# kerrm/vlite-fast

Measured on AMD Instinct MI355X. Metric: Msamp/s/antenna (dual-pol) and x real-time @128 MS/s; % HBM roofline, higher is better.
Workload: dtype f32

## Files before the change

### vlite-fast_amd/csrc/search_dev.h

```cpp
#pragma once
#include <hip/hip_runtime.h>

#include <cstdint>

#define GATHER_FLUSH 240

typedef uint32_t gather_u32x4 __attribute__((ext_vector_type(4), aligned(4)));

template <int NDW>
__device__ __forceinline__ void gather_load(const uint32_t *p, uint32_t (&w)[NDW + 1])
{
#pragma unroll
    for (int i = 0; i + 4 <= NDW + 1; i += 4) {
        const gather_u32x4 v = *(const gather_u32x4 *)(p + i);
        w[i] = v.x;
        w[i + 1] = v.y;
        w[i + 2] = v.z;
        w[i + 3] = v.w;
    }
#pragma unroll
    for (int i = (NDW + 1) & ~3; i <= NDW; ++i) w[i] = p[i];
}

template <int NDW>
__device__ __forceinline__ void gather_load_guarded(const uint8_t *xt, long long off, uint32_t (&w)[NDW + 1])
{
    if (off >= 0) {
        gather_load<NDW>((const uint32_t *)(xt + off), w);
    } else {
#pragma unroll
        for (int i = 0; i <= NDW; ++i)
            if (off + 4 * i >= 0) w[i] = *(const uint32_t *)(xt + off + 4 * i);
    }
}

__device__ __forceinline__ uint32_t gather_align(uint32_t w0, uint32_t w1, unsigned sh) { return __builtin_amdgcn_alignbyte(w1, w0, sh); }

template <int NDW>
__device__ __forceinline__ void gather_shift(const uint32_t (&w)[NDW + 1], unsigned sh, uint32_t (&a)[NDW])
{
#pragma unroll
    for (int i = 0; i < NDW; ++i) a[i] = gather_align(w[i], w[i + 1], sh);
}

#define SA_T 64
#define SA_B 64
#define SA_PITCH 84
#define SA_BPITCH 68

__device__ __forceinline__ void stream_store16(uint8_t *__restrict__ row, int td, int lo, int hi, const uint32_t (&w)[4])
{
    if (td >= lo && td + 16 <= hi) {
        *(uint4 *)(row + td) = make_uint4(w[0], w[1], w[2], w[3]);
        return;
    }
#pragma unroll
    for (int q = 0; q < 4; ++q) {
        const int tq = td + 4 * q;
        if (tq >= lo && tq + 4 <= hi) {
            *(uint32_t *)(row + tq) = w[q];
        } else {
#pragma unroll
            for (int k = 0; k < 4; ++k)
                if (tq + k >= lo && tq + k < hi) row[tq + k] = (uint8_t)(w[q] >> (8 * k));
        }
    }
}


template <typename T, typename Op>
__device__ __forceinline__ T block_reduce(T v, T *sh, T zero, Op op)
{
    for (int o = 32; o >= 1; o >>= 1) v = op(v, __shfl_down(v, o));
    __syncthreads();
    if ((threadIdx.x & 63) == 0) sh[threadIdx.x >> 6] = v;
    __syncthreads();
    T r = zero;
#pragma unroll
    for (int i = 0; i < 4; ++i) r = op(r, sh[i]);
    return r;
}

template <typename T>
__device__ __forceinline__ T block_sum(T v, T *sh)
{
    return block_reduce(v, sh, (T)0, [](T a, T b) { return a + b; });
}

__device__ __forceinline__ unsigned long long block_max(unsigned long long v, unsigned long long *sh)
{
    return block_reduce(v, sh, 0ull, [](unsigned long long a, unsigned long long b) { return b > a ? b : a; });
}

template <typename T>
__device__ __forceinline__ T wave_inclusive_sum(T v)
{
    const int lane = threadIdx.x & 63;
    for (int o = 1; o < 64; o <<= 1) {
        const T y = __shfl_up(v, o);
        if (lane >= o) v += y;
    }
    return v;
}

__device__ __forceinline__ int block_wave_offsets(int wave_total, int *sh, int &before)
{
    const int wave = threadIdx.x >> 6;
    __syncthreads();
    if ((threadIdx.x & 63) == 63) sh[wave] = wave_total;
    __syncthreads();
    int tot = 0;
    before = 0;
#pragma unroll
    for (int w = 0; w < 4; ++w) {
        if (w < wave) before += sh[w];
        tot += sh[w];
    }
    return tot;
}

__device__ __forceinline__ int block_count(bool flag, int *sh, int &rank)
{
    const uint64_t m = __ballot(flag);
    int before;
    const int tot = block_wave_offsets(__popcll(m), sh, before);
    rank = before + __popcll(m & ((1ull << (threadIdx.x & 63)) - 1ull));
    return tot;
}
```

### vlite-fast_amd/csrc/search_run.hip

```cpp
#include "search_internal.h"
#include "search_dev.h"

std::string g_search_err;

__global__ __launch_bounds__(256) void k_transpose_codes(const uint8_t *__restrict__ codes, uint8_t *__restrict__ xt,
                                                         int T, int nchan, int nbit, size_t tpitch)
{
    __shared__ uint8_t tile[64][65];
    const int t0 = blockIdx.x * 64, c0 = blockIdx.y * 64;
    const int per = 8 / nbit, maskv = (1 << nbit) - 1;
    for (int i = threadIdx.x; i < 64 * 64; i += 256) {
        const int tt = i / 64, cc = i % 64;
        const int t = t0 + tt, c = c0 + cc;
        uint8_t v = 0;
        if (t < T && c < nchan) {
            const size_t n = (size_t)t * nchan + c;
            v = (codes[n / per] >> (nbit * (n % per))) & maskv;
        }
        tile[tt][cc] = v;
    }
    __syncthreads();
    for (int i = threadIdx.x; i < 64 * 64; i += 256) {
        const int cc = i / 64, tt = i % 64;
        const int t = t0 + tt, c = c0 + cc;
        if (t < T && c < nchan) xt[(size_t)c * tpitch + t] = tile[tt][cc];
    }
}

#ifndef DDM_DB
#define DDM_DB 4
#endif
#ifndef DDM_SAMPLES
#define DDM_SAMPLES 8
#endif
#ifndef DDM_CU
#define DDM_CU 4
#endif
#define DDM_TILE (256 * DDM_SAMPLES)

__global__ __launch_bounds__(256) void k_dedisperse(const uint8_t *__restrict__ xt, const int32_t *__restrict__ chans,
                                                    const int32_t *__restrict__ delay, uint32_t *__restrict__ D,
                                                    int nact, int ndm, int tout, size_t tpitch, size_t dpitch)
{
    const int dm0 = blockIdx.y * DDM_DB;
    const int t = blockIdx.x * DDM_TILE + threadIdx.x * DDM_SAMPLES;
    if (t >= tout) return;
    uint32_t lo[DDM_DB][DDM_SAMPLES / 4], hi[DDM_DB][DDM_SAMPLES / 4];
    uint32_t acc[DDM_DB][DDM_SAMPLES];
    const int32_t *dl[DDM_DB];
#pragma unroll
    for (int j = 0; j < DDM_DB; ++j) {
        dl[j] = delay + (size_t)(dm0 + j < ndm ? dm0 + j : ndm - 1) * nact;
#pragma unroll
        for (int w = 0; w < DDM_SAMPLES / 4; ++w) lo[j][w] = hi[j][w] = 0u;
#pragma unroll
        for (int i = 0; i < DDM_SAMPLES; ++i) acc[j][i] = 0u;
    }
    auto flush = [&]() {
#pragma unroll
        for (int j = 0; j < DDM_DB; ++j) {
#pragma unroll
            for (int w = 0; w < DDM_SAMPLES / 4; ++w) {
                acc[j][4 * w + 0] += lo[j][w] & 0xffffu;
                acc[j][4 * w + 1] += hi[j][w] & 0xffffu;
                acc[j][4 * w + 2] += lo[j][w] >> 16;
                acc[j][4 * w + 3] += hi[j][w] >> 16;
                lo[j][w] = hi[j][w] = 0u;
            }
        }
    };
    auto fetch = [&](int c, int j, uint32_t (&w)[DDM_SAMPLES / 4 + 1], unsigned &sh) {
        const int32_t d = dl[j][c];
        const uint32_t *p = (const uint32_t *)(xt + (size_t)chans[c] * tpitch + t + (d & ~3));
#pragma unroll
        for (int i = 0; i <= DDM_SAMPLES / 4; ++i) w[i] = p[i];
        sh = (unsigned)(d & 3);
    };
    auto add = [&](int j, const uint32_t (&w)[DDM_SAMPLES / 4 + 1], unsigned sh) {
#pragma unroll
        for (int i = 0; i < DDM_SAMPLES / 4; ++i) {
            const uint32_t a = gather_align(w[i], w[i + 1], sh);
            lo[j][i] += a & 0x00ff00ffu;
            hi[j][i] += (a >> 8) & 0x00ff00ffu;
        }
    };
    int c = 0, since = 0;
    for (; c + DDM_CU <= nact; c += DDM_CU) {
        uint32_t w[DDM_CU][DDM_DB][DDM_SAMPLES / 4 + 1];
        unsigned sh[DDM_CU][DDM_DB];
#pragma unroll
        for (int u = 0; u < DDM_CU; ++u)
#pragma unroll
            for (int j = 0; j < DDM_DB; ++j) fetch(c + u, j, w[u][j], sh[u][j]);
#pragma unroll
        for (int u = 0; u < DDM_CU; ++u)
#pragma unroll
            for (int j = 0; j < DDM_DB; ++j) add(j, w[u][j], sh[u][j]);
        since += DDM_CU;
        if (since >= GATHER_FLUSH) {
            flush();
            since = 0;
        }
    }
    for (; c < nact; ++c) {
#pragma unroll
        for (int j = 0; j < DDM_DB; ++j) {
            uint32_t w[DDM_SAMPLES / 4 + 1];
            unsigned sh;
            fetch(c, j, w, sh);
            add(j, w, sh);
        }
    }
    flush();
#pragma unroll
    for (int j = 0; j < DDM_DB; ++j) {
        if (dm0 + j >= ndm) break;
        uint32_t *out = D + (size_t)(dm0 + j) * dpitch + t;
#pragma unroll
        for (int i = 0; i < DDM_SAMPLES; i += 4) {
            if (t + i + 4 <= tout) {
                *(uint4 *)(out + i) = make_uint4(acc[j][i], acc[j][i + 1], acc[j][i + 2], acc[j][i + 3]);
            } else {
                for (int q = 0; q < 4; ++q)
                    if (t + i + q < tout) out[i + q] = acc[j][i + q];
            }
        }
    }
}

__global__ __launch_bounds__(256) void k_prefix(const uint32_t *__restrict__ D, uint64_t *__restrict__ P, int tout,
                                                size_t dpitch, size_t ppitch)
{
    __shared__ uint64_t sh[256];
    const uint32_t *x = D + (size_t)blockIdx.x * dpitch;
    uint64_t *p = P + (size_t)blockIdx.x * ppitch;
    const int per = (tout + 255) / 256;
    const int lo = threadIdx.x * per, hi = min(lo + per, tout);
    uint64_t s = 0;
    for (int t = lo; t < hi; ++t) s += x[t];
    sh[threadIdx.x] = s;
    __syncthreads();
    if (threadIdx.x == 0) {
        uint64_t run = 0;
        for (int i = 0; i < 256; ++i) {
            const uint64_t v = sh[i];
            sh[i] = run;
            run += v;
        }
        p[0] = 0;
    }
    __syncthreads();
    uint64_t run = sh[threadIdx.x];
    for (int t = lo; t < hi; ++t) {
        run += x[t];
        p[t + 1] = run;
    }
}

__device__ __forceinline__ float baseline_at(const uint64_t *__restrict__ p, int t, int W, int tout, float gmean)
{
    if (W <= 0) return gmean;
    int lo = t - W / 2, hi = lo + W;
    if (lo < 0) { lo = 0; hi = min(W, tout); }
    if (hi > tout) { hi = tout; lo = max(0, tout - W); }
    return (float)((double)(p[hi] - p[lo]) / (double)(hi - lo));
}

__global__ __launch_bounds__(256) void k_series_stats(const uint32_t *__restrict__ D, const uint64_t *__restrict__ P,
                                                      float *__restrict__ stats, int tout, int W, size_t dpitch,
                                                      size_t ppitch)
{
    __shared__ double sh[4];
    const uint32_t *x = D + (size_t)blockIdx.x * dpitch;
    const uint64_t *p = P + (size_t)blockIdx.x * ppitch;
    const float gmean0 = (float)((double)p[tout] / (double)tout);
    double s1 = 0, s2 = 0;
    for (int t = threadIdx.x; t < tout; t += 256) {
        const double v = (double)x[t] - (double)baseline_at(p, t, W, tout, gmean0);
        s1 += v;
        s2 += v * v;
    }
    s1 = block_sum(s1, sh);
    s2 = block_sum(s2, sh);
    double mean = s1 / tout, var = s2 / tout - mean * mean;
    double rms = sqrt(var > 0 ? var : 0);
    const double mean1 = mean, rms1 = rms;
    double c1 = 0, cn = 0;
    for (int t = threadIdx.x; t < tout; t += 256) {
        const double v = (double)x[t] - (double)baseline_at(p, t, W, tout, gmean0);
        if (fabs(v - mean1) <= 3 * rms1) {
            c1 += v;
            cn += 1;
        }
    }
    c1 = block_sum(c1, sh);
    cn = block_sum(cn, sh);
    if (cn > 0) {
        mean = c1 / cn;
        double d2 = 0;
        for (int t = threadIdx.x; t < tout; t += 256) {
            const double v = (double)x[t] - (double)baseline_at(p, t, W, tout, gmean0);
            if (fabs(v - mean1) <= 3 * rms1) d2 += (v - mean) * (v - mean);
        }
        d2 = block_sum(d2, sh);
        rms = sqrt(d2 / cn / 0.97330);
    }
    if (threadIdx.x == 0) {
        stats[2 * blockIdx.x] = (float)(W > 0 ? mean : mean + (double)gmean0);
        stats[2 * blockIdx.x + 1] = (float)rms;
    }
}

__global__ __launch_bounds__(256) void k_boxcar(const uint64_t *__restrict__ P, const float *__restrict__ stats,
                                                float *__restrict__ snr, uint8_t *__restrict__ wid, int tout,
                                                int nbox, int W, size_t dpitch, size_t ppitch, float thresh,
                                                int32_t *__restrict__ peaks, int max_peaks)
{
    const int dm = blockIdx.y;
    const int t = blockIdx.x * 256 + threadIdx.x;
    if (t >= tout) return;
    const uint64_t *p = P + (size_t)dm * ppitch;
    const float lvl = stats[2 * dm], rms = stats[2 * dm + 1];
    float best = -1e30f;
    int bw = 0;
    for (int k = 0; k < nbox; ++k) {
        const int w = 1 << k;
        if (t + w > tout) break;
        const float sum = (float)(p[t + w] - p[t]);
        const float base = W > 0 ? baseline_at(p, t + w / 2, W, tout, 0.f) + lvl : lvl;
        const float sn = (sum - (float)w * base) / (rms * sqrtf((float)w));
        if (sn > best) {
            best = sn;
            bw = k;
        }
    }
    if (!(rms > 0)) best = 0.f;
    snr[(size_t)dm * dpitch + t] = best;
    wid[(size_t)dm * dpitch + t] = (uint8_t)bw;
    if (peaks && best >= thresh) {
        const int i = atomicAdd(peaks, 1);
        if (i < max_peaks) {
            peaks[1 + 4 * i] = dm;
            peaks[2 + 4 * i] = t;
            peaks[3 + 4 * i] = __float_as_int(best);
            peaks[4 + 4 * i] = bw;
        }
    }
}


__device__ __forceinline__ int first_bin_reaching(const uint32_t (&a)[4], uint32_t need)
{
    const int lane = threadIdx.x & 63;
    const uint32_t loc = a[0] + a[1] + a[2] + a[3];
    const uint32_t inc = wave_inclusive_sum(loc);
    const int first = __builtin_ctzll(__ballot(inc >= need));
    uint32_t c = inc - loc;
    int k = 3;
    for (int j = 0; j < 4; ++j) {
        c += a[j];
        if (c >= need) {
            k = j;
            break;
        }
    }
    return __shfl(4 * lane + k, first);
}

__global__ __launch_bounds__(256) void k_rfi_narrow(uint8_t *__restrict__ xt, const int32_t *__restrict__ chans,
                                                    uint8_t *__restrict__ med_out, int nsamp, size_t tpitch, float tol,
                                                    int replace, unsigned long long *__restrict__ nflag)
{
    __shared__ uint32_t hist[4][256];
    __shared__ uint32_t tot[256];
    __shared__ int sh_med, sh_mad;
    __shared__ uint32_t sh_cnt[4];
    const int wave = threadIdx.x >> 6, lane = threadIdx.x & 63;
    for (int i = threadIdx.x; i < 4 * 256; i += 256) hist[i >> 8][i & 255] = 0u;
    __syncthreads();
    uint8_t *row = xt + (size_t)chans[blockIdx.x] * tpitch;
    uint4 *rv = (uint4 *)row;
    const int nvec = nsamp >> 4;
    for (int i = threadIdx.x; i < nvec; i += 256) {
        const uint4 v = rv[i];
        const uint32_t w[4] = {v.x, v.y, v.z, v.w};
#pragma unroll
        for (int j = 0; j < 4; ++j)
#pragma unroll
            for (int b = 0; b < 4; ++b) atomicAdd(&hist[wave][(w[j] >> (8 * b)) & 255u], 1u);
    }
    for (int t = 16 * nvec + threadIdx.x; t < nsamp; t += 256) atomicAdd(&hist[wave][row[t]], 1u);
    __syncthreads();
    tot[threadIdx.x] = hist[0][threadIdx.x] + hist[1][threadIdx.x] + hist[2][threadIdx.x] + hist[3][threadIdx.x];
    __syncthreads();
    if (wave == 0) {
        const uint32_t need = (uint32_t)(nsamp + 1) / 2;
        uint32_t a[4];
#pragma unroll
        for (int j = 0; j < 4; ++j) a[j] = tot[4 * lane + j];
        const int med = first_bin_reaching(a, need);
#pragma unroll
        for (int j = 0; j < 4; ++j) {
            const int d = 4 * lane + j;
            a[j] = d == 0 ? tot[med] : (med - d >= 0 ? tot[med - d] : 0u) + (med + d < 256 ? tot[med + d] : 0u);
        }
        const int mad = first_bin_reaching(a, need);
        if (lane == 0) {
            sh_med = med;
            sh_mad = mad;
            med_out[blockIdx.x] = (uint8_t)med;
        }
    }
    __syncthreads();
    if (!replace) return;
    const int med = sh_med;
    const float thr = tol * 1.4826f * (float)max(sh_mad, 1);
    const int dlim = thr >= 255.f ? 255 : (int)floorf(thr);
    const uint32_t mb = (uint32_t)med;
    uint32_t cnt = 0;
    for (int i = threadIdx.x; i < nvec; i += 256) {
        const uint4 v = rv[i];
        uint32_t w[4] = {v.x, v.y, v.z, v.w};
        uint32_t changed = 0;
#pragma unroll
        for (int j = 0; j < 4; ++j) {
            uint32_t o = 0;
#pragma unroll
            for (int b = 0; b < 4; ++b) {
                const uint32_t x = (w[j] >> (8 * b)) & 255u;
                const bool f = abs((int)x - med) > dlim;
                cnt += f;
                changed |= f;
                o |= (f ? mb : x) << (8 * b);
            }
            w[j] = o;
        }
        if (changed) rv[i] = make_uint4(w[0], w[1], w[2], w[3]);
    }
    for (int t = 16 * nvec + threadIdx.x; t < nsamp; t += 256) {
        if (abs((int)row[t] - med) > dlim) {
            row[t] = (uint8_t)med;
            ++cnt;
        }
    }
    cnt = block_sum(cnt, sh_cnt);
    if (threadIdx.x == 0 && cnt) atomicAdd(nflag, (unsigned long long)cnt);
}

__global__ __launch_bounds__(256) void k_rfi_broad_list(const float *__restrict__ snr, const uint8_t *__restrict__ wid,
                                                        int nsamp, float tol, int widest, int32_t *__restrict__ tlist,
                                                        unsigned long long *__restrict__ nbroad)
{
    __shared__ int end[256 + 64];
    const int base = blockIdx.x * 256;
    for (int i = threadIdx.x; i < 256 + 64; i += 256) {
        const int t0 = base - 64 + i;
        int e = 0;
        if (t0 >= 0 && t0 < nsamp && snr[t0] >= tol) e = t0 + (1 << wid[t0]);
        end[i] = e;
    }
    __syncthreads();
    const int t = base + threadIdx.x;
    if (t >= nsamp) return;
    bool f = false;
    for (int k = 0; k < widest; ++k) f |= end[64 + threadIdx.x - k] > t;
    if (f) {
        const unsigned long long i = atomicAdd(nbroad, 1ull);
        tlist[i] = t;
    }
}

__global__ __launch_bounds__(256) void k_rfi_broad_mask(uint8_t *__restrict__ xt, const int32_t *__restrict__ chans,
                                                        const uint8_t *__restrict__ med, const int32_t *__restrict__ tlist,
                                                        const unsigned long long *__restrict__ nbroad, int nact,
                                                        size_t tpitch)
{
    const int k = blockIdx.x * 4 + (threadIdx.x >> 6);
    if (k >= nact) return;
    const int n = (int)*nbroad;
    uint8_t *row = xt + (size_t)chans[k] * tpitch;
    const uint8_t m = med[k];
    for (int i = threadIdx.x & 63; i < n; i += 64) row[tlist[i]] = m;
}

extern "C" const char *pb_search_last_error(const pb_search *s) { return s ? s->err.c_str() : g_search_err.c_str(); }

static int search_create(int device, int nchan, int max_samples, float fch1_mhz, float foff_mhz, float tsamp_s,
                         const std::vector<double> &dms, int boxcar_max, const int *zap_ranges, int nzap,
                         pb_search **out);

extern "C" int pb_search_create(int device, int nchan, int max_samples, float fch1_mhz, float foff_mhz, float tsamp_s,
                                float dm_min, float dm_max, float dm_step, int boxcar_max, const int *zap_ranges,
                                int nzap, pb_search **out)
{
    if (!out || !(dm_step > 0) || dm_max < dm_min) return search_fail(nullptr, "pb_search_create", "bad argument");
    const int ndm = (int)floor((dm_max - dm_min) / dm_step + 1e-6) + 1;
    std::vector<double> dms(ndm);
    for (int i = 0; i < ndm; ++i) dms[i] = (double)dm_min + (double)i * (double)dm_step;
    return search_create(device, nchan, max_samples, fch1_mhz, foff_mhz, tsamp_s, dms, boxcar_max, zap_ranges, nzap, out);
}

extern "C" int pb_search_create_list(int device, int nchan, int max_samples, float fch1_mhz, float foff_mhz,
                                     float tsamp_s, const float *dm_list, int ndm, int boxcar_max,
                                     const int *zap_ranges, int nzap, pb_search **out)
{
    if (!out || !dm_list || ndm < 1) return search_fail(nullptr, "pb_search_create_list", "bad argument");
    std::vector<double> dms(dm_list, dm_list + ndm);
    for (int i = 1; i < ndm; ++i)
        if (!(dms[i] > dms[i - 1])) return search_fail(nullptr, "pb_search_create_list", "the DM list must be strictly ascending");
    return search_create(device, nchan, max_samples, fch1_mhz, foff_mhz, tsamp_s, dms, boxcar_max, zap_ranges, nzap, out);
}

static int search_create(int device, int nchan, int max_samples, float fch1_mhz, float foff_mhz, float tsamp_s,
                         const std::vector<double> &dms, int boxcar_max, const int *zap_ranges, int nzap,
                         pb_search **out)
{
    const float dm_min = (float)dms.front();
    if (!out || nchan < 1 || max_samples < 64 || boxcar_max < 1) return search_fail(nullptr, "pb_search_create", "bad argument");
    if (!(dm_min >= 0) || device < 0) {
        g_search_err = "pb_search_create: dm_min and device must be >= 0";
        return PB_EINVAL;
    }
    *out = nullptr;
    int ndev = 0;
    if (hipGetDeviceCount(&ndev) != hipSuccess || ndev <= 0 || device >= ndev) {
        g_search_err = "pb_search_create: no HIP device (no CPU fallback)";
        return PB_EHIP;
    }
    pb_search *s = new pb_search();
    s->device = device;
    s->nchan = nchan;
    s->max_samples = max_samples;
    s->fch1 = fch1_mhz;
    s->foff = foff_mhz;
    s->tsamp = tsamp_s;
    s->ndm = (int)dms.size();
    while ((1 << s->nbox) <= boxcar_max) s->nbox++;
    s->dm_last = dms.back();
    std::vector<int32_t> chans;
    for (int c = 0; c < nchan; ++c) {
        bool zap = false;
        for (int z = 0; z < nzap; ++z)
            if (c >= zap_ranges[2 * z] && c < zap_ranges[2 * z + 1]) zap = true;
        if (!zap) chans.push_back(c);
    }
    s->nact = (int)chans.size();
    if (s->nact == 0) {
        g_search_err = "pb_search_create: every channel is zapped";
        delete s;
        return PB_EINVAL;
    }
    std::vector<int32_t> delay((size_t)s->ndm * s->nact);
    const double ftop = foff_mhz < 0 ? fch1_mhz : fch1_mhz + (nchan - 1) * foff_mhz;
    s->ftop = ftop;
    int maxd = 0;
    for (int i = 0; i < s->ndm; ++i) {
        const double dm = dms[i];
        for (int k = 0; k < s->nact; ++k) {
            const double f = (double)fch1_mhz + (double)chans[k] * (double)foff_mhz;
            const int32_t di = delay_samples(dm, delay_chan_term(f, ftop), (double)tsamp_s);
            delay[(size_t)i * s->nact + k] = di;
            if (di > maxd) maxd = di;
        }
    }
    s->max_delay = maxd;
    s->tpitch = ((size_t)max_samples + 63) / 64 * 64;
    hipError_t e = hipSetDevice(device);
    if (e == hipSuccess) e = hipStreamCreateWithFlags(&s->stream, hipStreamNonBlocking);
    if (e == hipSuccess) e = hipMalloc((void **)&s->d_codes, (size_t)max_samples * nchan);
    if (e == hipSuccess) e = hipMalloc((void **)&s->d_xt, s->tpitch * nchan + 64);
    if (e == hipSuccess) e = hipMemset(s->d_xt, 0, s->tpitch * nchan + 64);
    if (e == hipSuccess) e = hipMalloc((void **)&s->d_delay, delay.size() * sizeof(int32_t));
    if (e == hipSuccess) e = hipMalloc((void **)&s->d_chans, chans.size() * sizeof(int32_t));
    if (e == hipSuccess) e = hipMemcpy(s->d_chans, chans.data(), chans.size() * sizeof(int32_t), hipMemcpyHostToDevice);
    if (e == hipSuccess) e = hipMalloc((void **)&s->d_D, (size_t)s->ndm * s->tpitch * sizeof(uint32_t));
    if (e == hipSuccess) e = hipMalloc((void **)&s->d_stats, (size_t)s->ndm * 2 * sizeof(float));
    if (e == hipSuccess) e = hipMalloc((void **)&s->d_snr, (size_t)s->ndm * s->tpitch * sizeof(float));
    if (e == hipSuccess) e = hipMalloc((void **)&s->d_wid, (size_t)s->ndm * s->tpitch);
    if (e == hipSuccess) e = hipMalloc((void **)&s->d_P, (size_t)s->ndm * s->ppitch() * sizeof(uint64_t));
    if (e == hipSuccess) e = hipMalloc((void **)&s->d_peaks, (size_t)(1 + 4 * s->max_peaks) * sizeof(int32_t));
    for (int i = 0; i < 7 && e == hipSuccess; ++i) e = hipEventCreate(&s->ev[i]);
    if (e == hipSuccess) e = hipMemcpy(s->d_delay, delay.data(), delay.size() * sizeof(int32_t), hipMemcpyHostToDevice);
    if (e != hipSuccess) {
        g_search_err = std::string("pb_search_create: ") + hipGetErrorString(e);
        pb_search_destroy(s);
        return PB_EHIP;
    }
    *out = s;
    return PB_OK;
}

void search_rfi_free(pb_search *s)
{
    search_release({s->rfi.d_zdelay, s->rfi.d_med, s->rfi.d_z, s->rfi.d_zP, s->rfi.d_zstats, s->rfi.d_zsnr, s->rfi.d_zwid,
                    s->rfi.d_tlist, s->rfi.d_rcnt}, nullptr, s->rfi.ev, 1);
    s->rfi = {};
}

extern "C" void pb_search_destroy(pb_search *s)
{
    if (!s) return;
    (void)hipSetDevice(s->device);
    if (s->stream) (void)hipStreamSynchronize(s->stream);
    search_rfi_free(s);
    search_rfichan_free(s);
    search_cutouts_free(s);
    search_refine_free(s);
    search_giants_free(s);
    search_gulp_free(s);
    search_pol_free(s);
    search_subbands_free(s);
    search_release({s->d_codes, s->d_xt, s->d_delay, s->d_D, s->d_stats, s->d_snr, s->d_wid, s->d_P, s->d_peaks, s->d_chans},
                   nullptr, s->ev, 7);
    if (s->stream) (void)hipStreamDestroy(s->stream);
    delete s;
}

extern "C" int pb_search_info(const pb_search *s, int *ndm, int *nbox, int *max_delay)
{
    if (!s) return PB_EINVAL;
    if (ndm) *ndm = s->ndm;
    if (nbox) *nbox = s->nbox;
    if (max_delay) *max_delay = s->max_delay;
    return PB_OK;
}

extern "C" int pb_search_set_baseline(pb_search *s, int window_samples)
{
    if (!s || window_samples < 0) return PB_EINVAL;
    s->baseline = window_samples;
    return PB_OK;
}

extern "C" int pb_search_set_rfi(pb_search *s, int narrow, int broad, float tol, int rfi_boxcar_max)
{
    const char *fn = "pb_search_set_rfi";
    if (!(tol > 0) || !std::isfinite(tol)) return search_fail(s, fn, "tol must be > 0 and finite");
    if (rfi_boxcar_max < 1 || rfi_boxcar_max > 64 || (rfi_boxcar_max & (rfi_boxcar_max - 1)))
        return search_fail(s, fn, "rfi_boxcar_max must be a power of two in 1..64");
    if (!s) return search_fail(s, fn, "no search handle");
    if ((narrow || broad) && !s->rfi.d_rcnt) {
        const size_t tp = s->tpitch;
        SCHK(s, hipSetDevice(s->device));
        SCHK(s, hipMalloc((void **)&s->rfi.d_zdelay, (size_t)s->nact * sizeof(int32_t)));
        SCHK(s, hipMemset(s->rfi.d_zdelay, 0, (size_t)s->nact * sizeof(int32_t)));
        SCHK(s, hipMalloc((void **)&s->rfi.d_med, (size_t)s->nact));
        SCHK(s, hipMalloc((void **)&s->rfi.d_z, tp * sizeof(uint32_t)));
        SCHK(s, hipMalloc((void **)&s->rfi.d_zP, s->ppitch() * sizeof(uint64_t)));
        SCHK(s, hipMalloc((void **)&s->rfi.d_zstats, 2 * sizeof(float)));
        SCHK(s, hipMalloc((void **)&s->rfi.d_zsnr, tp * sizeof(float)));
        SCHK(s, hipMalloc((void **)&s->rfi.d_zwid, tp));
        SCHK(s, hipMalloc((void **)&s->rfi.d_tlist, tp * sizeof(int32_t)));
        SCHK(s, hipEventCreate(&s->rfi.ev[0]));
        SCHK(s, hipMalloc((void **)&s->rfi.d_rcnt, 2 * sizeof(unsigned long long)));
    }
    s->rfi.narrow = narrow != 0;
    s->rfi.broad = broad != 0;
    s->rfi.tol = tol;
    s->rfi.nbox = 0;
    while ((1 << s->rfi.nbox) <= rfi_boxcar_max) s->rfi.nbox++;
    return PB_OK;
}

static int search_clean(pb_search *s, int nsamp)
{
    const size_t ppitch = s->ppitch();
    SCHK(s, hipMemsetAsync(s->rfi.d_rcnt, 0, 2 * sizeof(unsigned long long), s->stream));
    k_rfi_narrow<<<s->nact, 256, 0, s->stream>>>(s->d_xt, s->d_chans, s->rfi.d_med, nsamp, s->tpitch, s->rfi.tol,
                                                 s->rfi.narrow, s->rfi.d_rcnt);
    if (s->rfi.broad) {
        dim3 gz((nsamp + DDM_TILE - 1) / DDM_TILE, 1);
        k_dedisperse<<<gz, 256, 0, s->stream>>>(s->d_xt, s->d_chans, s->rfi.d_zdelay, s->rfi.d_z, s->nact, 1, nsamp, s->tpitch,
                                                s->tpitch);
        k_prefix<<<1, 256, 0, s->stream>>>(s->rfi.d_z, s->rfi.d_zP, nsamp, s->tpitch, ppitch);
        k_series_stats<<<1, 256, 0, s->stream>>>(s->rfi.d_z, s->rfi.d_zP, s->rfi.d_zstats, nsamp, s->baseline, s->tpitch, ppitch);
        dim3 gb((nsamp + 255) / 256, 1);
        k_boxcar<<<gb, 256, 0, s->stream>>>(s->rfi.d_zP, s->rfi.d_zstats, s->rfi.d_zsnr, s->rfi.d_zwid, nsamp, s->rfi.nbox, s->baseline,
                                            s->tpitch, ppitch, 0.f, nullptr, 0);
        k_rfi_broad_list<<<gb, 256, 0, s->stream>>>(s->rfi.d_zsnr, s->rfi.d_zwid, nsamp, s->rfi.tol, 1 << (s->rfi.nbox - 1),
                                                    s->rfi.d_tlist, s->rfi.d_rcnt + 1);
        k_rfi_broad_mask<<<(s->nact + 3) / 4, 256, 0, s->stream>>>(s->d_xt, s->d_chans, s->rfi.d_med, s->rfi.d_tlist,
                                                                   s->rfi.d_rcnt + 1, s->nact, s->tpitch);
    }
    SCHK(s, hipEventRecord(s->rfi.ev[0], s->stream));
    return PB_OK;
}

void search_series_launch(pb_search *s, const uint32_t *D, uint64_t *P, float *stats, int nrow, int tout)
{
    k_prefix<<<nrow, 256, 0, s->stream>>>(D, P, tout, s->tpitch, s->ppitch());
    k_series_stats<<<nrow, 256, 0, s->stream>>>(D, P, stats, tout, s->baseline, s->tpitch, s->ppitch());
}

void search_boxcar_launch(pb_search *s, const uint64_t *P, const float *stats, float *snr, uint8_t *wid, int nrow, int tout)
{
    k_boxcar<<<dim3((tout + 255) / 256, nrow), 256, 0, s->stream>>>(P, stats, snr, wid, tout, s->nbox, s->baseline, s->tpitch,
                                                                    s->ppitch(), 0.f, nullptr, 0);
}

int search_block(pb_search *s, int nsamp, float thresh, bool want_peaks, bool cleaned)
{
    const int tout = nsamp - s->max_delay;
    s->rfi.ran = s->rfi.narrow || s->rfi.broad;
    s->chan.launched = s->chan.tol > 0 && !cleaned;
    s->chan.ran = s->chan.launched || (s->chan.tol > 0 && s->chan.have);
    if (s->chan.launched) {
        const int rc = search_rfichan_launch(s, nsamp);
        if (rc) return rc;
    }
    if (s->chan.tol > 0 && !s->rfi.ran) SCHK(s, hipEventRecord(s->chan.ev[2], s->stream));
    if (s->rfi.ran && cleaned) {
        SCHK(s, hipEventRecord(s->rfi.ev[0], s->stream));
    } else if (s->rfi.ran) {
        const int rc = search_clean(s, nsamp);
        if (rc) return rc;
    }
    dim3 gd((tout + 255) / 256, s->ndm);
    dim3 gdd((tout + DDM_TILE - 1) / DDM_TILE, (s->ndm + DDM_DB - 1) / DDM_DB);
    k_dedisperse<<<gdd, 256, 0, s->stream>>>(s->d_xt, s->d_chans, s->d_delay, s->d_D, s->nact, s->ndm, tout, s->tpitch, s->tpitch);
    SCHK(s, hipEventRecord(s->ev[3], s->stream));
    const size_t ppitch = s->ppitch();
    k_prefix<<<s->ndm, 256, 0, s->stream>>>(s->d_D, s->d_P, tout, s->tpitch, ppitch);
    k_series_stats<<<s->ndm, 256, 0, s->stream>>>(s->d_D, s->d_P, s->d_stats, tout, s->baseline, s->tpitch, ppitch);
    SCHK(s, hipEventRecord(s->ev[4], s->stream));
    if (want_peaks) SCHK(s, hipMemsetAsync(s->d_peaks, 0, sizeof(int32_t), s->stream));
    k_boxcar<<<gd, 256, 0, s->stream>>>(s->d_P, s->d_stats, s->d_snr, s->d_wid, tout, s->nbox, s->baseline, s->tpitch,
                                        ppitch, thresh, want_peaks ? s->d_peaks : nullptr, s->max_peaks);
    SCHK(s, hipEventRecord(s->ev[5], s->stream));
    SCHK(s, hipGetLastError());
    s->last_tout = tout;
    s->last_nsamp = nsamp;
    s->plane_tout = tout;
    return PB_OK;
}

static int search_run(pb_search *s, const void *codes, int codes_on_device, int nsamp, int nbit, float thresh,
                      bool want_peaks)
{
    if (!s || !codes) return PB_EINVAL;
    if (nsamp > s->max_samples || !(nbit == 8 || nbit == 4 || nbit == 2))
        return search_fail(s, "pb_search_run", "block too long or bad nbit");
    const int tout = nsamp - s->max_delay;
    if (tout < 64) return search_fail(s, "pb_search_run", "block shorter than the largest dispersion delay");
    SCHK(s, hipSetDevice(s->device));
    const bool pol = s->pol.max > 0;
    if (pol && nbit != 8) return search_fail(s, "pb_search_run", "with polarisation on the block must be 8-bit");
    const size_t nbytes = (size_t)nsamp * s->nchan * nbit / 8 * (pol ? 4 : 1);
    const uint8_t *d_codes = (const uint8_t *)codes;
    s->gp.fill = 0;
    s->gp.cleaned = 0;
    s->gp.tail_n = 0;
    SCHK(s, hipEventRecord(s->ev[0], s->stream));
    if (!codes_on_device) {
        uint8_t *stage = pol ? s->pol.d_codes : s->d_codes;
        SCHK(s, hipMemcpyAsync(stage, codes, nbytes, hipMemcpyHostToDevice, s->stream));
        d_codes = stage;
    }
    SCHK(s, hipEventRecord(s->ev[1], s->stream));
    if (pol) {
        const int rc = search_pol_transpose(s, d_codes, nsamp);
        if (rc) return rc;
    } else {
        dim3 gt((nsamp + 63) / 64, (s->nchan + 63) / 64);
        k_transpose_codes<<<gt, 256, 0, s->stream>>>(d_codes, s->d_xt, nsamp, s->nchan, nbit, s->tpitch);
    }
    SCHK(s, hipEventRecord(s->ev[2], s->stream));
    return search_block(s, nsamp, thresh, want_peaks, false);
}

static int search_times(pb_search *s)
{
    hipEvent_t dd = s->rfi.ran ? s->rfi.ev[0] : (s->chan.tol > 0 ? s->chan.ev[2] : s->ev[2]);
    for (int i = 0; i < 6; ++i) s->ms[i] = search_ms(i == 2 ? dd : s->ev[i], s->ev[i + 1]);
    s->rfi.n_narrow = 0;
    s->rfi.n_broad = 0;
    s->rfi.ms = 0.f;
    if (s->rfi.ran) {
        unsigned long long c[2];
        SCHK(s, hipMemcpy(c, s->rfi.d_rcnt, sizeof c, hipMemcpyDeviceToHost));
        s->rfi.n_narrow = c[0];
        s->rfi.n_broad = (int)c[1];
        s->rfi.ms = search_ms(s->chan.launched ? s->chan.ev[1] : s->ev[2], s->rfi.ev[0]);
    }
    return PB_OK;
}

int search_run_out(pb_search *s, float *snr, uint8_t *width_log2, uint32_t *series, float *stats, int *tout_out)
{
    const int tout = s->last_tout;
    SCHK(s, hipStreamSynchronize(s->stream));
    if (snr) SCHK(s, hipMemcpy2D(snr, tout * sizeof(float), s->d_snr, s->tpitch * sizeof(float), tout * sizeof(float), s->ndm, hipMemcpyDeviceToHost));
    if (width_log2) SCHK(s, hipMemcpy2D(width_log2, tout, s->d_wid, s->tpitch, tout, s->ndm, hipMemcpyDeviceToHost));
    if (series) SCHK(s, hipMemcpy2D(series, tout * sizeof(uint32_t), s->d_D, s->tpitch * sizeof(uint32_t), tout * sizeof(uint32_t), s->ndm, hipMemcpyDeviceToHost));
    if (stats) SCHK(s, hipMemcpy(stats, s->d_stats, (size_t)s->ndm * 2 * sizeof(float), hipMemcpyDeviceToHost));
    SCHK(s, hipEventRecord(s->ev[6], s->stream));
    SCHK(s, hipEventSynchronize(s->ev[6]));
    const int rc = search_times(s);
    if (rc) return rc;
    if (tout_out) *tout_out = tout;
    return PB_OK;
}

int search_peaks_out(pb_search *s, int32_t *peaks, int max_out, int *npeaks, int *tout_out)
{
    int32_t n = 0;
    SCHK(s, hipMemcpyAsync(&n, s->d_peaks, sizeof n, hipMemcpyDeviceToHost, s->stream));
    SCHK(s, hipStreamSynchronize(s->stream));
    const int ncopy = std::min(std::min((int)n, max_out), s->max_peaks);
    if (ncopy > 0) SCHK(s, hipMemcpy(peaks, s->d_peaks + 1, (size_t)ncopy * 4 * sizeof(int32_t), hipMemcpyDeviceToHost));
    SCHK(s, hipEventRecord(s->ev[6], s->stream));
    SCHK(s, hipEventSynchronize(s->ev[6]));
    const int rc = search_times(s);
    if (rc) return rc;
    *npeaks = n;
    if (tout_out) *tout_out = s->last_tout;
    return PB_OK;
}

extern "C" int pb_search_run(pb_search *s, const void *codes, int codes_on_device, int nsamp, int nbit, float *snr,
                             uint8_t *width_log2, uint32_t *series, float *stats, int *tout_out)
{
    const int rc = search_run(s, codes, codes_on_device, nsamp, nbit, 0.f, false);
    return rc ? rc : search_run_out(s, snr, width_log2, series, stats, tout_out);
}

extern "C" int pb_search_peaks(pb_search *s, const void *codes, int codes_on_device, int nsamp, int nbit,
                               float threshold, int32_t *peaks, int max_out, int *npeaks, int *tout_out)
{
    if (!peaks || !npeaks || max_out < 1) return PB_EINVAL;
    const int rc = search_run(s, codes, codes_on_device, nsamp, nbit, threshold, true);
    return rc ? rc : search_peaks_out(s, peaks, max_out, npeaks, tout_out);
}

extern "C" int pb_search_timers(const pb_search *s, float *ms6)
{
    return search_get_ms(s, s ? s->ms : nullptr, 6, ms6);
}

extern "C" int pb_search_rfi_info(const pb_search *s, uint64_t *n_narrow, int *n_broad_samples, float *ms)
{
    if (!s) return PB_EINVAL;
    if (n_narrow) *n_narrow = s->rfi.n_narrow;
    if (n_broad_samples) *n_broad_samples = s->rfi.n_broad;
    if (ms) *ms = s->rfi.ms;
    return PB_OK;
}

extern "C" int pb_search_fetch_clean(pb_search *s, uint8_t *xt, size_t nbytes)
{
    if (!s || !xt) return PB_EINVAL;
    const size_t n = s->last_nsamp;
    if (n == 0 || nbytes < n * s->nchan)
        return search_fail(s, "pb_search_fetch_clean", "no block searched yet, or the buffer is smaller than nchan x nsamp");
    SCHK(s, hipSetDevice(s->device));
    SCHK(s, hipStreamSynchronize(s->stream));
    SCHK(s, hipMemcpy2D(xt, n, s->d_xt, s->tpitch, n, s->nchan, hipMemcpyDeviceToHost));
    return PB_OK;
}
```

Baseline: 224,700.

## Restructure dedispersion gather with 16-byte vector loads, DPP neighbor exchange, and perm unpack

Each lane now covers 16 samples and loads them as one aligned 16-byte vector instead of five scalar words. The spill-over word is taken from the next lane's first word through a DPP row shift, with one extra scalar load only at the wavefront edge. Byte alignment plus masking is replaced by v_perm selectors that shift and unpack into 16-bit lanes in one step. DM-per-block and channel unroll are halved, and launch bounds now request occupancy 4. The aim is fewer memory instructions and fewer ALU ops per sample, at the cost of less reuse of each channel row across DMs and fragile DPP row-boundary semantics.

```diff
diff --git a/vlite-fast_amd/csrc/search_dev.h b/vlite-fast_amd/csrc/search_dev.h
--- a/vlite-fast_amd/csrc/search_dev.h
+++ b/vlite-fast_amd/csrc/search_dev.h
@@ -35,6 +35,20 @@
 }
 
 __device__ __forceinline__ uint32_t gather_align(uint32_t w0, uint32_t w1, unsigned sh) { return __builtin_amdgcn_alignbyte(w1, w0, sh); }
+
+__device__ __forceinline__ uint32_t gather_sel_lo(unsigned sh) { return 0x0c020c00u + sh * 0x00010001u; }
+__device__ __forceinline__ uint32_t gather_sel_hi(unsigned sh) { return 0x0c030c01u + sh * 0x00010001u; }
+__device__ __forceinline__ void gather_unpack16(uint32_t w0, uint32_t w1, uint32_t sel_lo, uint32_t sel_hi, uint32_t &lo,
+                                                uint32_t &hi)
+{
+    lo = __builtin_amdgcn_perm(w1, w0, sel_lo);
+    hi = __builtin_amdgcn_perm(w1, w0, sel_hi);
+}
+
+__device__ __forceinline__ uint32_t gather_next_lane(uint32_t w0, uint32_t edge)
+{
+    return (uint32_t)__builtin_amdgcn_update_dpp((int)edge, (int)w0, 0x130, 0xf, 0xf, false);
+}
 
 template <int NDW>
 __device__ __forceinline__ void gather_shift(const uint32_t (&w)[NDW + 1], unsigned sh, uint32_t (&a)[NDW])
diff --git a/vlite-fast_amd/csrc/search_run.hip b/vlite-fast_amd/csrc/search_run.hip
--- a/vlite-fast_amd/csrc/search_run.hip
+++ b/vlite-fast_amd/csrc/search_run.hip
@@ -27,24 +27,23 @@
     }
 }
 
-#ifndef DDM_DB
-#define DDM_DB 4
-#endif
-#ifndef DDM_SAMPLES
-#define DDM_SAMPLES 8
-#endif
-#ifndef DDM_CU
-#define DDM_CU 4
-#endif
+#define DDM_DB 2
+#define DDM_SAMPLES 16
+#define DDM_CU 2
+#define DDM_NDW (DDM_SAMPLES / 4)
 #define DDM_TILE (256 * DDM_SAMPLES)
-
-__global__ __launch_bounds__(256) void k_dedisperse(const uint8_t *__restrict__ xt, const int32_t *__restrict__ chans,
-                                                    const int32_t *__restrict__ delay, uint32_t *__restrict__ D,
-                                                    int nact, int ndm, int tout, size_t tpitch, size_t dpitch)
+static_assert(DDM_NDW == 4, "k_dedisperse loads a lane's samples as one 16-byte vector");
+
+__global__ __launch_bounds__(256, 4) void k_dedisperse(const uint8_t *__restrict__ xt, const int32_t *__restrict__ chans,
+                                                       const int32_t *__restrict__ delay, uint32_t *__restrict__ D,
+                                                       int nact, int ndm, int tout, size_t tpitch, size_t dpitch)
 {
     const int dm0 = blockIdx.y * DDM_DB;
     const int t = blockIdx.x * DDM_TILE + threadIdx.x * DDM_SAMPLES;
     if (t >= tout) return;
+    const int lane = threadIdx.x & 63;
+    const int nlive = min(64, (tout - (t - lane * DDM_SAMPLES) + DDM_SAMPLES - 1) / DDM_SAMPLES);
+    const int t_edge = t + (nlive - lane) * DDM_SAMPLES;
     uint32_t lo[DDM_DB][DDM_SAMPLES / 4], hi[DDM_DB][DDM_SAMPLES / 4];
     uint32_t acc[DDM_DB][DDM_SAMPLES];
     const int32_t *dl[DDM_DB];
@@ -69,29 +68,35 @@
             }
         }
     };
-    auto fetch = [&](int c, int j, uint32_t (&w)[DDM_SAMPLES / 4 + 1], unsigned &sh) {
+    auto fetch = [&](const uint8_t *row, int c, int j, uint32_t (&w)[DDM_NDW + 1], unsigned &sh) {
         const int32_t d = dl[j][c];
-        const uint32_t *p = (const uint32_t *)(xt + (size_t)chans[c] * tpitch + t + (d & ~3));
-#pragma unroll
-        for (int i = 0; i <= DDM_SAMPLES / 4; ++i) w[i] = p[i];
+        const gather_u32x4 v = *(const gather_u32x4 *)(row + (uint32_t)(t + (d & ~3)));
+        w[0] = v.x, w[1] = v.y, w[2] = v.z, w[3] = v.w;
+        w[DDM_NDW] = *(const uint32_t *)(row + (uint32_t)(t_edge + (d & ~3)));
         sh = (unsigned)(d & 3);
     };
-    auto add = [&](int j, const uint32_t (&w)[DDM_SAMPLES / 4 + 1], unsigned sh) {
-#pragma unroll
-        for (int i = 0; i < DDM_SAMPLES / 4; ++i) {
-            const uint32_t a = gather_align(w[i], w[i + 1], sh);
-            lo[j][i] += a & 0x00ff00ffu;
-            hi[j][i] += (a >> 8) & 0x00ff00ffu;
+    auto add = [&](int j, const uint32_t (&w)[DDM_NDW + 1], unsigned sh) {
+        const uint32_t sel_lo = gather_sel_lo(sh), sel_hi = gather_sel_hi(sh);
+        const uint32_t wn = gather_next_lane(w[0], w[DDM_NDW]);
+#pragma unroll
+        for (int i = 0; i < DDM_NDW; ++i) {
+            uint32_t a, b;
+            gather_unpack16(w[i], i + 1 < DDM_NDW ? w[i + 1] : wn, sel_lo, sel_hi, a, b);
+            lo[j][i] += a;
+            hi[j][i] += b;
         }
     };
+    const uint32_t tp = (uint32_t)tpitch;
     int c = 0, since = 0;
     for (; c + DDM_CU <= nact; c += DDM_CU) {
-        uint32_t w[DDM_CU][DDM_DB][DDM_SAMPLES / 4 + 1];
+        uint32_t w[DDM_CU][DDM_DB][DDM_NDW + 1];
         unsigned sh[DDM_CU][DDM_DB];
 #pragma unroll
-        for (int u = 0; u < DDM_CU; ++u)
-#pragma unroll
-            for (int j = 0; j < DDM_DB; ++j) fetch(c + u, j, w[u][j], sh[u][j]);
+        for (int u = 0; u < DDM_CU; ++u) {
+            const uint8_t *row = xt + (uint64_t)(uint32_t)chans[c + u] * tp;
+#pragma unroll
+            for (int j = 0; j < DDM_DB; ++j) fetch(row, c + u, j, w[u][j], sh[u][j]);
+        }
 #pragma unroll
         for (int u = 0; u < DDM_CU; ++u)
 #pragma unroll
@@ -103,11 +108,12 @@
         }
     }
     for (; c < nact; ++c) {
+        const uint8_t *row = xt + (uint64_t)(uint32_t)chans[c] * tp;
 #pragma unroll
         for (int j = 0; j < DDM_DB; ++j) {
-            uint32_t w[DDM_SAMPLES / 4 + 1];
+            uint32_t w[DDM_NDW + 1];
             unsigned sh;
-            fetch(c, j, w, sh);
+            fetch(row, c, j, w, sh);
             add(j, w, sh);
         }
     }
```

Result: no change. 224,700 (-0.0%).
